# amada/PRT

Hardware: AMD Instinct MI355X
Metric: Mray/s (primary+secondary) at 1080p/64spp; 1/2/4/8-GPU scaling (higher is better)
Workload: dtype f32; 1 GPU; c3_sponza_standin; width=1920, height=1080, spp=64, max_depth=8, seed=12345, device=AMD Radeon Graphics, compute_units=256

## Files before the change

### prt_amd/csrc/prt_device.h

```cpp
#pragma once
#include <hip/hip_runtime.h>
#include <stdint.h>

#include "prt_devmath.h"
#include "prt_stats.h"

#define PRT_MAX_BVH 8
#ifndef PRT_STACK_LDS
#define PRT_STACK_LDS 12
#endif
#ifndef PRT_STACK_LDS_PACKET
#define PRT_STACK_LDS_PACKET (PRT_STACK_LDS / 2)
#endif
#define PRT_STACK_MAX 64
#ifndef PRT_BLOCK
#define PRT_BLOCK 1024
#endif
#define PRT_MAT_STRIDE 5
#ifndef PRT_IDLE_BREAK
#define PRT_IDLE_BREAK 24
#endif
#ifndef PRT_IDLE_BREAK_SCATTER
#define PRT_IDLE_BREAK_SCATTER PRT_IDLE_BREAK
#endif
#ifndef PRT_IDLE_BREAK_OCC
#define PRT_IDLE_BREAK_OCC PRT_IDLE_BREAK
#endif
struct DevScene {
    const float4* wnodes;
    const float4* hotNodes;
    const float* tris;
    const uint32_t* triAlpha;
    const uint32_t* triPrim;
    const float4* shade;
    const float4* bump;
    const float4* mats;
    const float4* alpha;
    const uint32_t* alphaClass;
    const uint4* texDesc;
    const uint8_t* texels;
    uint32_t bvhCount;
    uint32_t rootRef[PRT_MAX_BVH];
    float rootBox[PRT_MAX_BVH][6];
    uint32_t primBase[PRT_MAX_BVH];
    uint32_t hasNormals[PRT_MAX_BVH];
    uint32_t hasLight;
    float lightDir[3];
    float lightIntensity[3];
    float radius;
    uint32_t hasEnv;
    int32_t envW, envH, envFirstY;
    const float4* envTexels;
    const float* envV;
    const float* envHor;
    const int32_t* envFirstX;
};

struct DevCamera {
    float pos[3], dir[3], up[3], right[3];
    uint32_t width, height;
    float invWidth, invHeight;
};

struct Vec3 {
    float x, y, z;
};
struct Vec2 {
    float x, y;
};

__device__ __forceinline__ Vec3 mk3(float x, float y, float z) { return Vec3{x, y, z}; }
__device__ __forceinline__ Vec3 add3(Vec3 a, Vec3 b) { return mk3(a.x + b.x, a.y + b.y, a.z + b.z); }
__device__ __forceinline__ Vec3 sub3(Vec3 a, Vec3 b) { return mk3(a.x - b.x, a.y - b.y, a.z - b.z); }
__device__ __forceinline__ Vec3 mul3(Vec3 a, Vec3 b) { return mk3(a.x * b.x, a.y * b.y, a.z * b.z); }
__device__ __forceinline__ Vec3 div3s(Vec3 a, float s) { return mk3(a.x / s, a.y / s, a.z / s); }
__device__ __forceinline__ Vec3 scale3(float f, Vec3 v) { return mk3(f * v.x, f * v.y, f * v.z); }
__device__ __forceinline__ float dot3(Vec3 a, Vec3 b) { return a.x * b.x + a.y * b.y + a.z * b.z; }
__device__ __forceinline__ Vec3 cross3(Vec3 a, Vec3 b)
{
    return mk3(a.y * b.z - a.z * b.y, a.z * b.x - a.x * b.z, a.x * b.y - a.y * b.x);
}
__device__ __forceinline__ float length3(Vec3 v) { return sqrtf(dot3(v, v)); }
__device__ __forceinline__ Vec3 normalize3(Vec3 v)
{
    float invlen = 1.0f / length3(v);
    return scale3(invlen, v);
}
__device__ __forceinline__ float sse_min(float a, float b) { return a < b ? a : b; }
__device__ __forceinline__ float sse_max(float a, float b) { return a > b ? a : b; }
__device__ __forceinline__ float std_max(float a, float b) { return (a < b) ? b : a; }
__device__ __forceinline__ float asf(uint32_t u) { return __uint_as_float(u); }
__device__ __forceinline__ uint32_t asu(float f) { return __float_as_uint(f); }
__device__ __forceinline__ bool finite3(Vec3 v)
{
    return (asu(v.x) & 0x7f800000u) != 0x7f800000u && (asu(v.y) & 0x7f800000u) != 0x7f800000u && (asu(v.z) & 0x7f800000u) != 0x7f800000u;
}

#define PRT_AS1 __attribute__((address_space(1)))
typedef float prt_f4 __attribute__((ext_vector_type(4)));
typedef float prt_f3 __attribute__((ext_vector_type(3)));
typedef prt_f3 prt_f3u __attribute__((aligned(4)));
typedef uint32_t prt_u4 __attribute__((ext_vector_type(4)));
typedef uint32_t prt_u2 __attribute__((ext_vector_type(2)));
__device__ __forceinline__ float4 gld4(const float4* p)
{
    prt_f4 v = *(const PRT_AS1 prt_f4*)p;
    return make_float4(v.x, v.y, v.z, v.w);
}
__device__ __forceinline__ uint4 gld4u(const uint4* p)
{
    prt_u4 v = *(const PRT_AS1 prt_u4*)p;
    return make_uint4(v.x, v.y, v.z, v.w);
}
__device__ __forceinline__ uint2 gld2u(const uint2* p)
{
    prt_u2 v = *(const PRT_AS1 prt_u2*)p;
    return make_uint2(v.x, v.y);
}
__device__ __forceinline__ uint32_t gld(const uint32_t* p) { return *(const PRT_AS1 uint32_t*)p; }
__device__ __forceinline__ int32_t gld(const int32_t* p) { return *(const PRT_AS1 int32_t*)p; }
__device__ __forceinline__ float gld(const float* p) { return *(const PRT_AS1 float*)p; }
__device__ __forceinline__ uint32_t gld(const uint8_t* p) { return (uint32_t) * (const PRT_AS1 uint8_t*)p; }
__device__ __forceinline__ Vec3 ld3(const float* p, uint32_t v)
{
    const float* q = p + 3 * (size_t)v;
    return mk3(gld(q), gld(q + 1), gld(q + 2));
}
__device__ __forceinline__ void gst(uint32_t* p, uint32_t v) { *(PRT_AS1 uint32_t*)p = v; }
__device__ __forceinline__ void gst4(float4* p, float4 v)
{
    prt_f4 w = {v.x, v.y, v.z, v.w};
    *(PRT_AS1 prt_f4*)p = w;
}
__device__ __forceinline__ void gst2u(uint2* p, uint2 v)
{
    prt_u2 w = {v.x, v.y};
    *(PRT_AS1 prt_u2*)p = w;
}

struct DevRay {
    Vec3 org, dir, inv;
    bool swapXZ, swapYZ;
    bool fast;
    float invDz, shearX, shearY;
};

__device__ __forceinline__ void prepare_shear(DevRay& r)
{
    Vec3 d = r.dir;
    if (r.swapXZ) { float t = d.x; d.x = d.z; d.z = t; }
    if (r.swapYZ) { float t = d.y; d.y = d.z; d.z = t; }
    r.invDz = 1.0f / d.z;
    r.shearX = d.x * r.invDz;
    r.shearY = d.y * r.invDz;
    const float big = 3.402823466e+38f;
    r.fast = (fabsf(r.inv.x) <= big) && (fabsf(r.inv.y) <= big) && (fabsf(r.inv.z) <= big) && (fabsf(r.org.x) <= big) &&
             (fabsf(r.org.y) <= big) && (fabsf(r.org.z) <= big);
}

struct DevHit {
    float t, i, j, k;
    uint32_t primId, meshId;
};

struct Traffic {
    unsigned long long nBox, nTri;
    uint32_t nHit, nTap;
    [[no_unique_address]] TraceTally prof;
};

__device__ __forceinline__ void prepare_single(DevRay& r)
{
    r.inv = mk3(1.0f / r.dir.x, 1.0f / r.dir.y, 1.0f / r.dir.z);
    uint32_t e;
    if (r.dir.x > r.dir.y) e = (r.dir.x > r.dir.z) ? 0u : 2u;
    else e = (r.dir.y > r.dir.z) ? 1u : 2u;
    r.swapXZ = (e == 0u);
    r.swapYZ = (e == 1u);
    prepare_shear(r);
}

__device__ __forceinline__ void prepare_soa(DevRay& r)
{
    r.inv = mk3(1.0f / r.dir.x, 1.0f / r.dir.y, 1.0f / r.dir.z);
    float ax = fabsf(r.dir.x), ay = fabsf(r.dir.y), az = fabsf(r.dir.z);
    float max_e = sse_max(ax, sse_max(ay, az));
    bool mx = (max_e == ax);
    r.swapXZ = mx;
    r.swapYZ = (max_e == ay) && !mx;
    prepare_shear(r);
}

struct Box {
    Vec3 lo, hi;
};

template <bool FAST>
__device__ __forceinline__ float bmin(float a, float b) { return FAST ? __builtin_fminf(a, b) : (a < b ? a : b); }
template <bool FAST>
__device__ __forceinline__ float bmax(float a, float b) { return FAST ? __builtin_fmaxf(a, b) : (a > b ? a : b); }

template <bool FAST>
__device__ __forceinline__ void slabs(const Box& b, const DevRay& r, float t0[3], float t1[3])
{
    float a, c;
    a = (b.lo.x - r.org.x) * r.inv.x; c = (b.hi.x - r.org.x) * r.inv.x; t0[0] = bmin<FAST>(a, c); t1[0] = bmax<FAST>(a, c);
    a = (b.lo.y - r.org.y) * r.inv.y; c = (b.hi.y - r.org.y) * r.inv.y; t0[1] = bmin<FAST>(a, c); t1[1] = bmax<FAST>(a, c);
    a = (b.lo.z - r.org.z) * r.inv.z; c = (b.hi.z - r.org.z) * r.inv.z; t0[2] = bmin<FAST>(a, c); t1[2] = bmax<FAST>(a, c);
}

template <bool FAST>
__device__ __forceinline__ float box_t_impl(const Box& b, const DevRay& r)
{
    float t0[3], t1[3];
    slabs<FAST>(b, r, t0, t1);
    const float inf = __builtin_inff();
    float max_t0 = bmax<FAST>(bmax<FAST>(t0[0], t0[2]), bmax<FAST>(t0[1], -inf));
    float min_t1 = bmin<FAST>(bmin<FAST>(t1[0], t1[2]), bmin<FAST>(t1[1], inf));
    return (min_t1 < max_t0) ? inf : max_t0;
}
__device__ __forceinline__ float box_t(const Box& b, const DevRay& r) { return r.fast ? box_t_impl<true>(b, r) : box_t_impl<false>(b, r); }

template <bool FAST>
__device__ __forceinline__ bool box_bool_impl(const Box& b, const DevRay& r, float maxT)
{
    float t0[3], t1[3];
    slabs<FAST>(b, r, t0, t1);
    const float lowest = -3.402823466e+38f;
    float w0 = sse_min(lowest, maxT), w1 = sse_max(lowest, maxT);
    float max_t0 = bmax<FAST>(bmax<FAST>(t0[0], t0[2]), bmax<FAST>(t0[1], w0));
    float min_t1 = bmin<FAST>(bmin<FAST>(t1[0], t1[2]), bmin<FAST>(t1[1], w1));
    return min_t1 > max_t0;
}
__device__ __forceinline__ bool box_bool(const Box& b, const DevRay& r, float maxT)
{
    return r.fast ? box_bool_impl<true>(b, r, maxT) : box_bool_impl<false>(b, r, maxT);
}

template <bool FAST>
__device__ __forceinline__ float box_soa_entry_impl(const Box& b, const DevRay& r)
{
    float t0[3], t1[3];
    slabs<FAST>(b, r, t0, t1);
    float max_t0 = bmax<FAST>(t0[0], bmax<FAST>(t0[1], t0[2]));
    float min_t1 = bmin<FAST>(t1[0], bmin<FAST>(t1[1], t1[2]));
    return (min_t1 >= max_t0) ? max_t0 : __builtin_inff();
}
__device__ __forceinline__ float box_soa_entry(const Box& b, const DevRay& r)
{
    return r.fast ? box_soa_entry_impl<true>(b, r) : box_soa_entry_impl<false>(b, r);
}
__device__ __forceinline__ bool box_soa(const Box& b, const DevRay& r, float maxT) { return box_soa_entry(b, r) < maxT; }

__device__ __forceinline__ float slab_entry_select(const Box& b, const DevRay& r)
{
    float a, c, m, v;
    a = (b.lo.x - r.org.x) * r.inv.x; c = (b.hi.x - r.org.x) * r.inv.x; m = (a < c) ? a : c;
    a = (b.lo.y - r.org.y) * r.inv.y; c = (b.hi.y - r.org.y) * r.inv.y; v = (a < c) ? a : c; m = (v > m) ? v : m;
    a = (b.lo.z - r.org.z) * r.inv.z; c = (b.hi.z - r.org.z) * r.inv.z; v = (a < c) ? a : c; m = (v > m) ? v : m;
    return m;
}

__device__ __forceinline__ float tri_intersect(const DevRay& r, Vec3 p0, Vec3 p1, Vec3 p2, float& bi, float& bj, float& bk)
{
    Vec3 v0 = sub3(p0, r.org), v1 = sub3(p1, r.org), v2 = sub3(p2, r.org);
    if (r.swapXZ) {
        float t;
        t = v0.x; v0.x = v0.z; v0.z = t;
        t = v1.x; v1.x = v1.z; v1.z = t;
        t = v2.x; v2.x = v2.z; v2.z = t;
    }
    if (r.swapYZ) {
        float t;
        t = v0.y; v0.y = v0.z; v0.z = t;
        t = v1.y; v1.y = v1.z; v1.z = t;
        t = v2.y; v2.y = v2.z; v2.z = t;
    }
    float v0z = v0.z, v1z = v1.z, v2z = v2.z;
    const float inv_dz = r.invDz, idx = r.shearX, idy = r.shearY;
    float v0x = v0.x - idx * v0z, v0y = v0.y - idy * v0z;
    float v1x = v1.x - idx * v1z, v1y = v1.y - idy * v1z;
    float v2x = v2.x - idx * v2z, v2y = v2.y - idy * v2z;
    float e0 = v1x * v2y - v1y * v2x;
    float e1 = v2x * v0y - v2y * v0x;
    float e2 = v0x * v1y - v0y * v1x;
    bool mask_eb = (e0 < 0.0f || e1 < 0.0f || e2 < 0.0f) && (e0 > 0.0f || e1 > 0.0f || e2 > 0.0f);
    bi = bj = bk = 0.0f;
    if (mask_eb) return -1.0f;
    float det = e0 + e1 + e2;
    bool mask = (det < 0.0f) || (det > 0.0f);
    float inv_det = 1.0f / det;
    float t_scaled = (e0 * v0z + e1 * v1z + e2 * v2z) * inv_dz;
    float t = t_scaled * inv_det;
    mask = mask && (t > 0.0001f);
    bi = e0 * inv_det;
    bj = e1 * inv_det;
    bk = e2 * inv_det;
    return mask ? t : -1.0f;
}

__device__ __forceinline__ bool bilinear_cell(Vec2 uv, int32_t width, int32_t height, bool soa, int32_t& x0, int32_t& y0, float& xt, float& yt)
{
    float s = uv.x - floorf(uv.x);
    float t = uv.y - floorf(uv.y);
    if (soa) {
        xt = sse_max(s * (float)width - 0.5f, 0.0f);
        yt = sse_max(t * (float)height - 0.5f, 0.0f);
    } else {
        xt = std_max(s * (float)width - 0.5f, 0.0f);
        yt = std_max(t * (float)height - 0.5f, 0.0f);
    }
    x0 = (int32_t)floorf(xt);
    y0 = (int32_t)floorf(yt);
    return s == s && t == t;
}

__device__ __forceinline__ void bilinear(float k[4], int32_t idx[4], int32_t component, Vec2 uv, int32_t width, int32_t height, bool soa)
{
    float xt, yt;
    int32_t x0, y0;
    (void)bilinear_cell(uv, width, height, soa, x0, y0, xt, yt);
    int32_t x1 = (x0 + 1 < width - 1) ? x0 + 1 : width - 1;
    int32_t y1 = (y0 + 1 < height - 1) ? y0 + 1 : height - 1;
    idx[0] = component * (x0 + y0 * width);
    idx[1] = component * (x1 + y0 * width);
    idx[2] = component * (x0 + y1 * width);
    idx[3] = component * (x1 + y1 * width);
    const float s = xt - (float)x0;
    const float t = yt - (float)y0;
    k[0] = (1.0f - s) * (1.0f - t);
    k[1] = s * (1.0f - t);
    k[2] = (1.0f - s) * t;
    k[3] = s * t;
}

template <bool COUNT>
__device__ __forceinline__ bool tex_test_alpha(const DevScene& sc, uint4 d, Vec2 uv, bool soa, Traffic& tr)
{
    const uint8_t* p = sc.texels + d.x;
    float k[4];
    int32_t idx[4];
    bilinear(k, idx, (int32_t)d.w, uv, (int32_t)d.y, (int32_t)d.z, soa);
    if (COUNT) tr.nTap++;
    float alpha = 0.0f;
#pragma unroll
    for (int i = 0; i < 4; i++) alpha = alpha + k[i] * (float)gld(p + idx[i] + 3);
    return alpha > 127.0f;
}

template <bool SOA>
__device__ __forceinline__ bool alpha_decide(const DevScene& sc, const uint4& d, const float& classBits, const Vec2& uv, Traffic& tr)
{
    int32_t x0, y0;
    float xt, yt;
    uint32_t cls = 0u;
    if (bilinear_cell(uv, (int32_t)d.y, (int32_t)d.z, SOA, x0, y0, xt, yt)) {
        const uint32_t cell = (uint32_t)x0 + (uint32_t)y0 * d.y;
        cls = (gld(sc.alphaClass + asu(classBits) + (cell >> 4)) >> ((cell & 15u) * 2u)) & 3u;
    }
    bool pass;
    if (cls == 0u) pass = tex_test_alpha<false>(sc, d, uv, SOA, tr);
    else pass = cls == 1u;
    return pass;
}

template <bool COUNT>
__device__ __forceinline__ Vec3 tex_sample3(const DevScene& sc, uint4 d, Vec2 uv, Traffic& tr)
{
    const uint8_t* p = sc.texels + d.x;
    float k[4];
    int32_t idx[4];
    bilinear(k, idx, (int32_t)d.w, uv, (int32_t)d.y, (int32_t)d.z, false);
    if (COUNT) tr.nTap++;
    Vec3 c = mk3(0.0f, 0.0f, 0.0f);
#pragma unroll
    for (int i = 0; i < 4; i++) {
        const uint8_t* q = p + idx[i];
        c = add3(c, scale3(k[i], mk3((float)gld(q), (float)gld(q + 1), (float)gld(q + 2))));
    }
    return scale3(1.0f / 255.0f, c);
}

template <bool COUNT>
__device__ __forceinline__ float tex_sample1(const DevScene& sc, uint4 d, Vec2 uv, Traffic& tr)
{
    const uint8_t* p = sc.texels + d.x;
    float k[4];
    int32_t idx[4];
    bilinear(k, idx, (int32_t)d.w, uv, (int32_t)d.y, (int32_t)d.z, false);
    if (COUNT) tr.nTap++;
    float c = 0.0f;
#pragma unroll
    for (int i = 0; i < 4; i++) c = c + k[i] * (float)gld(p + idx[i]);
    return (1.0f / 255.0f) * c;
}

#define PRT_REF_LEAF 0x80000000u
#define PRT_LEAF_ALPHA 8u
__device__ __forceinline__ uint32_t leaf_count(uint32_t ref) { return (ref & 7u) + 1u; }
__device__ __forceinline__ uint32_t leaf_first(uint32_t ref) { return (ref >> 4) & 0x7ffffffu; }
__device__ __forceinline__ void load_tri(const DevScene& sc, uint32_t tri, Vec3& p0, Vec3& p1, Vec3& p2)
{
    const float* tp = sc.tris + 9 * (size_t)tri;
    const prt_f3 a = *(const PRT_AS1 prt_f3u*)tp, b = *(const PRT_AS1 prt_f3u*)(tp + 3), c = *(const PRT_AS1 prt_f3u*)(tp + 6);
    p0 = mk3(a.x, a.y, a.z);
    p1 = mk3(b.x, b.y, b.z);
    p2 = mk3(c.x, c.y, c.z);
}
#define PRT_REF_HOT 0x40000000u
#ifndef PRT_HOT_NODES
#define PRT_HOT_NODES 256
#endif

typedef __attribute__((address_space(3))) uint32_t lds_u32;
typedef __attribute__((address_space(3))) float lds_f32;
typedef __attribute__((address_space(3))) prt_f4 lds_f4;
template <int NLDS>
struct StackT {
    static constexpr int kLds = NLDS;
    lds_u32* ldsRef;
    lds_f32* ldsT;
    uint32_t* spillBase;
    uint32_t spillStride;
    const lds_f4* hot;
    lds_u32* coop;
    __device__ __forceinline__ uint32_t* deep(int e, int word) const
    {
        uint32_t thread;
        asm volatile("v_lshrrev_b32 %0, 2, %1" : "=v"(thread) : "v"((uint32_t)(uintptr_t)ldsRef - (uint32_t)(uintptr_t)(ldsRef - threadIdx.x)));
        return spillBase + ((size_t)(2 * (e - NLDS) + word) * spillStride + (blockIdx.x * PRT_BLOCK + thread));
    }
    __device__ __forceinline__ void put(int e, uint32_t ref) const
    {
        if (e < NLDS) ldsRef[e * PRT_BLOCK] = ref;
        else gst(deep(e, 0), ref);
    }
    __device__ __forceinline__ uint32_t get(int e) const
    {
        uint32_t v = ldsRef[(e < NLDS ? e : 0) * PRT_BLOCK];
        if (e >= NLDS) v = gld(deep(e, 0));
        return v;
    }
    __device__ __forceinline__ void putT(int e, uint32_t ref, float t) const
    {
        if (e < NLDS) {
            ldsRef[e * PRT_BLOCK] = ref;
            ldsT[e * PRT_BLOCK] = t;
        } else {
            gst(deep(e, 0), ref);
            gst(deep(e, 1), asu(t));
        }
    }
    __device__ __forceinline__ float getT(int e) const
    {
        float v = ldsT[(e < NLDS ? e : 0) * PRT_BLOCK];
        if (e >= NLDS) v = asf(gld(deep(e, 1)));
        return v;
    }
};

typedef float f2_t __attribute__((ext_vector_type(2)));

struct WideNode {
    float4 w0, w1, w2;
    uint32_t ref0, ref1, axis;
    __device__ __forceinline__ Box box0() const { return Box{mk3(w0.x, w0.z, w1.x), mk3(w0.y, w0.w, w1.y)}; }
    __device__ __forceinline__ Box box1() const { return Box{mk3(w2.x, w2.z, w1.z), mk3(w2.y, w2.w, w1.w)}; }
};

template <class STK>
__device__ __forceinline__ void load_wide(const DevScene& sc, const STK& st, uint32_t idx, WideNode& w)
{
    float4 w3;
    if (st.hot != nullptr && (idx & PRT_REF_HOT)) {
        const lds_f4* h = st.hot + 4u * (idx & (PRT_HOT_NODES - 1u));
        const prt_f4 a = h[0], b = h[1], c = h[2], d = h[3];
        w.w0 = make_float4(a.x, a.y, a.z, a.w);
        w.w1 = make_float4(b.x, b.y, b.z, b.w);
        w.w2 = make_float4(c.x, c.y, c.z, c.w);
        w3 = make_float4(d.x, d.y, d.z, d.w);
    } else {
        const float4* p = (idx & PRT_REF_HOT) ? sc.hotNodes + 4u * (idx & (PRT_HOT_NODES - 1u)) : sc.wnodes + 4 * (size_t)idx;
        w.w0 = gld4(p);
        w.w1 = gld4(p + 1);
        w.w2 = gld4(p + 2);
        w3 = gld4(p + 3);
    }
    w.ref0 = asu(w3.x);
    w.ref1 = asu(w3.y);
    w.axis = asu(w3.z);
}

__device__ __forceinline__ Box root_box(const DevScene& sc, uint32_t m)
{
    return Box{mk3(sc.rootBox[m][0], sc.rootBox[m][1], sc.rootBox[m][2]), mk3(sc.rootBox[m][3], sc.rootBox[m][4], sc.rootBox[m][5])};
}

template <bool OCCLUDE, bool PACKET, bool COUNT>
__device__ __forceinline__ bool tri_candidate(const DevScene& sc, uint32_t tri, bool leafHasAlpha, uint32_t meshId, const DevRay& r, float limit, DevHit& hit,
                                              Traffic& tr)
{
    Vec3 p0, p1, p2;
    load_tri(sc, tri, p0, p1, p2);
    float bi, bj, bk;
    float t = tri_intersect(r, p0, p1, p2, bi, bj, bk);
    if (!(t >= 0.0001f && t < limit)) return false;
    const uint32_t alphaRef = leafHasAlpha ? gld(sc.triAlpha + tri) : 0u;
    if (alphaRef) {
        const float4* ap = sc.alpha + 3 * (size_t)(alphaRef - 1);
        float4 u0 = gld4(ap), u1 = gld4(ap + 1), u2 = gld4(ap + 2);
        Vec2 uv = Vec2{bi * u0.x + bj * u0.z + bk * u1.x, bi * u0.y + bj * u0.w + bk * u1.y};
        if (!tex_test_alpha<COUNT>(sc, make_uint4(asu(u2.x), asu(u2.y), asu(u2.z), asu(u2.w)), uv, PACKET, tr)) return false;
    }
    if (!OCCLUDE) {
        hit.t = t;
        hit.i = bi;
        hit.j = bj;
        hit.k = bk;
        hit.primId = tri;
        hit.meshId = meshId;
    }
    return true;
}

#define PRT_MODE_PACKET 0
#define PRT_MODE_SINGLE 1
#define PRT_MODE_OCC_PACKET 2
#define PRT_MODE_OCC_SINGLE 3
#define PRT_REF_NONE 0xfffffffeu

struct Tracer {
    DevRay r;
    float maxT;
    DevHit hit;
    uint32_t ref;
    int sp;
    uint32_t m;
    uint32_t rev;
    bool occ;
};

template <int MODE>
__device__ __forceinline__ void tracer_begin(Tracer& T, Vec3 org, Vec3 dir, float maxT, uint32_t rev)
{
    T.r.org = org;
    T.r.dir = dir;
    if (MODE == PRT_MODE_PACKET || MODE == PRT_MODE_OCC_PACKET) prepare_soa(T.r);
    else prepare_single(T.r);
    T.maxT = maxT;
    T.hit.t = maxT;
    T.hit.i = T.hit.j = T.hit.k = 0.0f;
    T.hit.primId = 0;
    T.hit.meshId = 0;
    T.ref = PRT_REF_NONE;
    T.sp = 0;
    T.m = 0xffffffffu;
    T.rev = rev;
    T.occ = false;
}

template <int MODE, bool COUNT, class STK>
__device__ __forceinline__ uint32_t tracer_pop(Tracer& T, const STK& st, Traffic& tr)
{
    if (MODE == PRT_MODE_PACKET) {
        while (T.sp > 0) {
            --T.sp;
            if (st.getT(T.sp) < T.hit.t) return st.get(T.sp);
        }
        return PRT_REF_NONE;
    } else {
        if (T.sp == 0) return PRT_REF_NONE;
        tr.prof.pop(T.sp - 1 >= STK::kLds);
        return st.get(--T.sp);
    }
}

template <int MODE, bool COUNT>
__device__ __forceinline__ bool tracer_next_bvh(const DevScene& sc, Tracer& T, Traffic& tr)
{
    for (;;) {
        T.m++;
        if (T.m >= sc.bvhCount) return false;
        if (COUNT) tr.nBox++;
        const uint32_t mu = (uint32_t)__builtin_amdgcn_readfirstlane((int)T.m);
        Box rb;
        uint32_t rootRef;
        if (__ballot(T.m != mu) == 0ull) {
            rb = root_box(sc, mu);
            rootRef = sc.rootRef[mu];
        } else {
            rb = root_box(sc, T.m);
            rootRef = sc.rootRef[T.m];
        }
        bool pass;
        if (MODE == PRT_MODE_PACKET) pass = box_soa(rb, T.r, T.hit.t);
        else if (MODE == PRT_MODE_SINGLE) pass = box_bool(rb, T.r, T.hit.t);
        else if (MODE == PRT_MODE_OCC_PACKET) pass = box_soa(rb, T.r, T.maxT);
        else pass = box_bool(rb, T.r, T.maxT);
        if (pass) {
            T.ref = rootRef;
            T.sp = 0;
            return true;
        }
    }
}

template <int MODE, bool COUNT, class STK>
__device__ __forceinline__ void tracer_any_hit_order(Tracer& T, const STK& st, Traffic& tr, const WideNode& w, bool h0, bool h1, bool near0)
{
    if (h0 && h1) {
        st.put(T.sp++, near0 ? w.ref1 : w.ref0);
        T.ref = near0 ? w.ref0 : w.ref1;
    } else if (h0) {
        T.ref = w.ref0;
    } else if (h1) {
        T.ref = w.ref1;
    } else {
        T.ref = tracer_pop<MODE, COUNT>(T, st, tr);
    }
}

struct NodeExt {
    float mx0, mn0, mx1, mn1;
};

template <int MODE, bool COUNT, class STK>
__device__ __forceinline__ void tracer_decide(const DevScene& sc, Tracer& T, const STK& st, Traffic& tr, const WideNode& w, const NodeExt& e)
{
    const float inf = __builtin_inff();
    if (MODE == PRT_MODE_SINGLE) {
        if (COUNT) tr.nBox += 2;
        float t0 = (e.mn0 < e.mx0) ? inf : e.mx0, t1 = (e.mn1 < e.mx1) ? inf : e.mx1;
        bool h0 = t0 < T.hit.t, h1 = t1 < T.hit.t;
        if (h0 && h1) {
            bool near0 = t0 < t1;
            st.put(T.sp++, near0 ? w.ref1 : w.ref0);
            T.ref = near0 ? w.ref0 : w.ref1;
        } else if (h0) {
            T.ref = w.ref0;
        } else if (h1) {
            T.ref = w.ref1;
        } else {
            T.ref = tracer_pop<MODE, COUNT>(T, st, tr);
        }
    } else if (MODE == PRT_MODE_PACKET) {
        if (COUNT) tr.nBox += 2;
        float e0 = (e.mn0 >= e.mx0) ? e.mx0 : inf, e1 = (e.mn1 >= e.mx1) ? e.mx1 : inf;
        bool rev = (T.rev >> (w.axis & 3u)) & 1u;
        uint32_t firstRef = rev ? w.ref1 : w.ref0, laterRef = rev ? w.ref0 : w.ref1;
        float firstE = rev ? e1 : e0, laterE = rev ? e0 : e1;
        if (laterE < T.hit.t) st.putT(T.sp++, laterRef, laterE);
        if (firstE < T.hit.t) T.ref = firstRef;
        else T.ref = tracer_pop<MODE, COUNT>(T, st, tr);
    } else {
        bool h0, h1;
        if (MODE == PRT_MODE_OCC_PACKET) {
            h0 = ((e.mn0 >= e.mx0) ? e.mx0 : inf) < T.maxT;
            h1 = ((e.mn1 >= e.mx1) ? e.mx1 : inf) < T.maxT;
        } else {
            const float lowest = -3.402823466e+38f;
            float w0 = sse_min(lowest, T.maxT), w1 = sse_max(lowest, T.maxT);
            h0 = __builtin_fminf(e.mn0, w1) > __builtin_fmaxf(e.mx0, w0);
            h1 = __builtin_fminf(e.mn1, w1) > __builtin_fmaxf(e.mx1, w0);
        }
        if (COUNT) tr.nBox += 2;
        tracer_any_hit_order<MODE, COUNT>(T, st, tr, w, h0, h1, e.mx0 <= e.mx1);
    }
}

template <int MODE, bool COUNT, class STK>
__device__ __forceinline__ void tracer_node(const DevScene& sc, Tracer& T, const STK& st, Traffic& tr, uint32_t& overflow)
{
    WideNode w;
    load_wide(sc, st, T.ref, w);
    if (T.sp + 2 >= PRT_STACK_MAX) {
        overflow = 1;
        T.ref = PRT_REF_NONE;
        T.sp = 0;
        T.m = sc.bvhCount;
        return;
    }
    if (T.r.fast) {
        const DevRay& r = T.r;
        const f2_t c0x = (f2_t{w.w0.x, w.w0.y} - r.org.x) * r.inv.x, c0y = (f2_t{w.w0.z, w.w0.w} - r.org.y) * r.inv.y;
        const f2_t c0z = (f2_t{w.w1.x, w.w1.y} - r.org.z) * r.inv.z, c1z = (f2_t{w.w1.z, w.w1.w} - r.org.z) * r.inv.z;
        const f2_t c1x = (f2_t{w.w2.x, w.w2.y} - r.org.x) * r.inv.x, c1y = (f2_t{w.w2.z, w.w2.w} - r.org.y) * r.inv.y;
        NodeExt e;
        e.mx0 = __builtin_fmaxf(__builtin_fmaxf(__builtin_fminf(c0x.x, c0x.y), __builtin_fminf(c0y.x, c0y.y)), __builtin_fminf(c0z.x, c0z.y));
        e.mn0 = __builtin_fminf(__builtin_fminf(__builtin_fmaxf(c0x.x, c0x.y), __builtin_fmaxf(c0y.x, c0y.y)), __builtin_fmaxf(c0z.x, c0z.y));
        e.mx1 = __builtin_fmaxf(__builtin_fmaxf(__builtin_fminf(c1x.x, c1x.y), __builtin_fminf(c1y.x, c1y.y)), __builtin_fminf(c1z.x, c1z.y));
        e.mn1 = __builtin_fminf(__builtin_fminf(__builtin_fmaxf(c1x.x, c1x.y), __builtin_fmaxf(c1y.x, c1y.y)), __builtin_fmaxf(c1z.x, c1z.y));
        tracer_decide<MODE, COUNT>(sc, T, st, tr, w, e);
        return;
    }
    const Box wb0 = w.box0(), wb1 = w.box1();
    if (MODE == PRT_MODE_SINGLE) {
        if (COUNT) tr.nBox += 2;
        float t0 = box_t(wb0, T.r), t1 = box_t(wb1, T.r);
        bool h0 = t0 < T.hit.t, h1 = t1 < T.hit.t;
        if (h0 && h1) {
            bool near0 = t0 < t1;
            st.put(T.sp++, near0 ? w.ref1 : w.ref0);
            T.ref = near0 ? w.ref0 : w.ref1;
        } else if (h0) {
            T.ref = w.ref0;
        } else if (h1) {
            T.ref = w.ref1;
        } else {
            T.ref = tracer_pop<MODE, COUNT>(T, st, tr);
        }
    } else if (MODE == PRT_MODE_PACKET) {
        if (COUNT) tr.nBox += 2;
        float e0 = box_soa_entry(wb0, T.r), e1 = box_soa_entry(wb1, T.r);
        bool rev = (T.rev >> (w.axis & 3u)) & 1u;
        uint32_t firstRef = rev ? w.ref1 : w.ref0, laterRef = rev ? w.ref0 : w.ref1;
        float firstE = rev ? e1 : e0, laterE = rev ? e0 : e1;
        if (laterE < T.hit.t) st.putT(T.sp++, laterRef, laterE);
        if (firstE < T.hit.t) T.ref = firstRef;
        else T.ref = tracer_pop<MODE, COUNT>(T, st, tr);
    } else {
        bool h0 = (MODE == PRT_MODE_OCC_PACKET) ? box_soa(wb0, T.r, T.maxT) : box_bool(wb0, T.r, T.maxT);
        bool h1 = (MODE == PRT_MODE_OCC_PACKET) ? box_soa(wb1, T.r, T.maxT) : box_bool(wb1, T.r, T.maxT);
        if (COUNT) tr.nBox += 2;
        tracer_any_hit_order<MODE, COUNT>(T, st, tr, w, h0, h1, slab_entry_select(wb0, T.r) <= slab_entry_select(wb1, T.r));
    }
}

template <int MODE, bool COUNT, class STK>
__device__ __forceinline__ void tracer_tri(const DevScene& sc, Tracer& T, const STK& st, Traffic& tr)
{
    constexpr bool OCC = (MODE == PRT_MODE_OCC_PACKET || MODE == PRT_MODE_OCC_SINGLE);
    constexpr bool PACKET = (MODE == PRT_MODE_PACKET || MODE == PRT_MODE_OCC_PACKET);
    const uint32_t left = leaf_count(T.ref), tri = leaf_first(T.ref);
    const bool hasAlpha = (T.ref & PRT_LEAF_ALPHA) != 0u;
    {
        if (COUNT) tr.nTri++;
        if (tri_candidate<OCC, PACKET, COUNT>(sc, tri, hasAlpha, T.m, T.r, OCC ? T.maxT : T.hit.t, T.hit, tr) && OCC) {
            T.occ = true;
            T.ref = PRT_REF_NONE;
            T.sp = 0;
            T.m = sc.bvhCount;
            return;
        }
    }
    if (left > 1u) {
        if (COUNT) tr.nTri++;
        if (tri_candidate<OCC, PACKET, COUNT>(sc, tri + 1u, hasAlpha, T.m, T.r, OCC ? T.maxT : T.hit.t, T.hit, tr) && OCC) {
            T.occ = true;
            T.ref = PRT_REF_NONE;
            T.sp = 0;
            T.m = sc.bvhCount;
            return;
        }
    }
    if (left > 2u) T.ref += 30u;
    else T.ref = tracer_pop<MODE, COUNT>(T, st, tr);
}

#ifndef PRT_COOP_MIN
#define PRT_COOP_MIN 9u
#endif
#ifndef PRT_COOP_WEIGHT
#define PRT_COOP_WEIGHT 4u
#endif
#define PRT_COOP_TRI_BITS 26

__device__ __forceinline__ uint32_t mbcnt64(unsigned long long m)
{
    return __builtin_amdgcn_mbcnt_hi((uint32_t)(m >> 32), __builtin_amdgcn_mbcnt_lo((uint32_t)m, 0u));
}

#define PRT_COOP_STRIDE 72u
#define PRT_COOP_TRI_MASK ((1u << PRT_COOP_TRI_BITS) - 1u)
__device__ __forceinline__ float bperm(int byteAddr, float v) { return __int_as_float(__builtin_amdgcn_ds_bpermute(byteAddr, __float_as_int(v))); }
__device__ __forceinline__ uint32_t bperm(int byteAddr, uint32_t v) { return (uint32_t)__builtin_amdgcn_ds_bpermute(byteAddr, (int)v); }

template <int MODE, class STK>
__device__ __forceinline__ void tracer_leaf_coop(const DevScene& sc, Tracer& T, bool onLeaf, const STK& st, Traffic& tr)
{
    constexpr bool OCC = (MODE == PRT_MODE_OCC_PACKET || MODE == PRT_MODE_OCC_SINGLE);
    constexpr bool PACKET = (MODE == PRT_MODE_PACKET || MODE == PRT_MODE_OCC_PACKET);
    const uint32_t lane = threadIdx.x & 63u;
    const uint32_t n = onLeaf ? leaf_count(T.ref) : 0u;
    const unsigned long long b0 = __ballot((n & 1u) != 0u), b1 = __ballot((n & 2u) != 0u), b2 = __ballot((n & 4u) != 0u), b3 = __ballot((n & 8u) != 0u);
    const uint32_t prefix = mbcnt64(b0) + 2u * mbcnt64(b1) + 4u * mbcnt64(b2) + 8u * mbcnt64(b3);
    const bool take = onLeaf && prefix + n <= 64u;
    const unsigned long long takeMask = __ballot(take);
    const uint32_t last = 63u - (uint32_t)__builtin_clzll(takeMask);
    const uint32_t pairs = (uint32_t)__builtin_amdgcn_readlane((int)(prefix + n), (int)last);
    tr.prof.leaf_pairs(pairs);
    {
        const uint32_t word = (((T.ref >> 4) - prefix) & PRT_COOP_TRI_MASK) | (lane << PRT_COOP_TRI_BITS);
        lds_u32* q = st.coop + (take ? prefix : 64u);
        const uint32_t nm1 = take ? n - 1u : 0u;
        q[0] = word;
#pragma unroll
        for (uint32_t i = 1; i < 8u; i++) q[i < nm1 ? i : nm1] = word;
    }
    __builtin_amdgcn_fence(__ATOMIC_ACQ_REL, "wavefront");
    const bool pair = lane < pairs;
    const uint32_t word = st.coop[lane];
    const int popAt = T.sp > 0 ? T.sp - 1 : 0;
    uint32_t popped = st.ldsRef[(popAt < STK::kLds ? popAt : 0) * PRT_BLOCK];
    const int oaddr = (int)((pair ? (word >> PRT_COOP_TRI_BITS) : lane) << 2);
    const uint32_t tri = (word + lane) & PRT_COOP_TRI_MASK;
    __builtin_amdgcn_sched_barrier(0);
    prt_f3 a, b, c;
    if (pair) {
        const float* tp = sc.tris + 9 * (size_t)tri;
        a = *(const PRT_AS1 prt_f3u*)tp;
        b = *(const PRT_AS1 prt_f3u*)(tp + 3);
        c = *(const PRT_AS1 prt_f3u*)(tp + 6);
    }
    __builtin_amdgcn_sched_barrier(0);
    DevRay r;
    r.org = mk3(bperm(oaddr, T.r.org.x), bperm(oaddr, T.r.org.y), bperm(oaddr, T.r.org.z));
    r.shearX = bperm(oaddr, T.r.shearX);
    r.shearY = bperm(oaddr, T.r.shearY);
    r.invDz = bperm(oaddr, T.r.invDz);
    const uint32_t flags = bperm(oaddr, (T.r.swapXZ ? 1u : 0u) | (T.r.swapYZ ? 2u : 0u) | ((T.ref & PRT_LEAF_ALPHA) ? 4u : 0u));
    const float limit = bperm(oaddr, OCC ? T.maxT : T.hit.t);
    __builtin_amdgcn_sched_barrier(0);
    r.swapXZ = (flags & 1u) != 0u;
    r.swapYZ = (flags & 2u) != 0u;
    float t = -1.0f, bi = 0.0f, bj = 0.0f, bk = 0.0f;
    uint32_t primId = 0u;
    bool cand = false;
    if (pair) {
        t = tri_intersect(r, mk3(a.x, a.y, a.z), mk3(b.x, b.y, b.z), mk3(c.x, c.y, c.z), bi, bj, bk);
        primId = tri;
        cand = t >= 0.0001f && t < limit;
        tr.prof.alpha_begin();
        const uint32_t alphaRef = (cand && (flags & 4u)) ? gld(sc.triAlpha + tri) : 0u;
        if (alphaRef) {
            const float4* ap = sc.alpha + 3 * (size_t)(alphaRef - 1);
            const float4 u0 = gld4(ap), u1 = gld4(ap + 1), u2 = gld4(ap + 2);
            const Vec2 uv = Vec2{bi * u0.x + bj * u0.z + bk * u1.x, bi * u0.y + bj * u0.w + bk * u1.y};
            const uint4 d = make_uint4(asu(u2.x), asu(u2.y), asu(u2.z), asu(u2.w));
            cand = alpha_decide<PACKET>(sc, d, u1.w, uv, tr);
        }
        tr.prof.alpha_end(cand, (flags & 4u) != 0u);
    }
    const unsigned long long acc = __ballot(cand);
    uint32_t seg = take ? ((uint32_t)(acc >> prefix) & ((1u << n) - 1u)) : 0u;
    if (OCC) {
        if (take) {
            if (seg) {
                T.occ = true;
                T.ref = PRT_REF_NONE;
                T.sp = 0;
                T.m = sc.bvhCount;
            } else {
                if (T.sp == 0) T.ref = PRT_REF_NONE;
                else {
                    if (popAt >= STK::kLds) popped = st.get(popAt);
                    T.sp = popAt;
                    T.ref = popped;
                }
            }
        }
    } else {
        if (acc != 0ull) {
            uint32_t win = 0xffffffffu;
            for (;;) {
                tr.prof.leaf_update();
                const bool more = seg != 0u;
                if (!__any(more)) break;
                const uint32_t src = more ? prefix + (uint32_t)__builtin_ctz(seg) : lane;
                const float t2 = bperm((int)(src << 2), t);
                if (more) {
                    if (t2 < T.hit.t) {
                        T.hit.t = t2;
                        win = src;
                    }
                    seg &= seg - 1u;
                }
            }
            if (__any(win != 0xffffffffu)) {
                const int waddr = (int)((win != 0xffffffffu ? win : lane) << 2);
                const float i2 = bperm(waddr, bi), j2 = bperm(waddr, bj), k2 = bperm(waddr, bk);
                const uint32_t p2 = bperm(waddr, primId);
                if (win != 0xffffffffu) {
                    T.hit.i = i2;
                    T.hit.j = j2;
                    T.hit.k = k2;
                    T.hit.primId = p2;
                    T.hit.meshId = T.m;
                }
            }
        }
        if (take) {
            if (MODE == PRT_MODE_PACKET) T.ref = tracer_pop<MODE, false>(T, st, tr);
            else if (T.sp == 0) T.ref = PRT_REF_NONE;
            else {
                if (popAt >= STK::kLds) popped = st.get(popAt);
                T.sp = popAt;
                T.ref = popped;
            }
        }
    }
}

__device__ __forceinline__ bool ref_is_internal(uint32_t ref) { return !(ref & PRT_REF_LEAF); }
__device__ __forceinline__ bool ref_is_leaf(uint32_t ref) { return (ref & PRT_REF_LEAF) && ref != PRT_REF_NONE; }

__device__ __forceinline__ constexpr uint32_t idle_break(int mode)
{
    return mode == 1 ? (uint32_t)(PRT_IDLE_BREAK_SCATTER) : mode >= 2 ? (uint32_t)(PRT_IDLE_BREAK_OCC) : (uint32_t)(PRT_IDLE_BREAK);
}
template <int MODE, bool COUNT, class STK>
__device__ __forceinline__ void trace_step_phase(const DevScene& sc, Tracer& T, bool active, const STK& st, Traffic& tr, uint32_t& overflow)
{
    for (;;) {
        const bool onNode = active && ref_is_internal(T.ref);
        const bool onLeaf = active && ref_is_leaf(T.ref);
        const uint32_t nNode = (uint32_t)__popcll(__ballot(onNode)), nLeaf = (uint32_t)__popcll(__ballot(onLeaf));
        if (nNode + nLeaf == 0u) break;
        const bool doNode = !COUNT ? (nLeaf == 0u || (nLeaf < PRT_COOP_MIN && nLeaf * PRT_COOP_WEIGHT < nNode)) : nNode >= nLeaf;
#ifdef PRT_PAD_VALU
        {
            float pad = T.maxT;
#pragma unroll
            for (int q = 0; q < PRT_PAD_VALU; q++) asm volatile("v_add_f32 %0, %0, %0" : "+v"(pad));
            asm volatile("" ::"v"(pad));
        }
#endif
        tr.prof.round(doNode, T.ref, onNode, onLeaf, active && T.ref == PRT_REF_NONE, active, nNode, nLeaf, COUNT);
        if (doNode) {
            tr.prof.node_begin(T.sp);
            if (onNode) tracer_node<MODE, COUNT>(sc, T, st, tr, overflow);
            tr.prof.node_end(onNode && ref_is_internal(T.ref) && !(T.ref & PRT_REF_HOT), T.sp);
        } else if (!COUNT) {
            tracer_leaf_coop<MODE>(sc, T, onLeaf, st, tr);
        } else {
            if (onLeaf) tracer_tri<MODE, COUNT>(sc, T, st, tr);
        }
        const uint32_t done = (uint32_t)__popcll(__ballot(active && T.ref == PRT_REF_NONE));
        if (done >= idle_break(MODE)) break;
    }
}

template <int MODE, bool COUNT, class Src, class STK>
__device__ __forceinline__ void trace_loop(const DevScene& sc, Src& src, const STK& st, Traffic& tr, uint32_t& overflow)
{
    const uint32_t n = src.count();
    const uint32_t lane = threadIdx.x & 63u;
    Tracer T{};
    T.ref = PRT_REF_NONE;
    T.sp = 0;
    T.m = 0;
    bool active = false, exhausted = false;
    uint32_t item = 0;
    const uint32_t totalWaves = gridDim.x * (PRT_BLOCK / 64);
    uint32_t chunk = n / (totalWaves * 4u);
    chunk = chunk < 64u ? 64u : (chunk > 1024u ? 1024u : chunk);
    if (n == 0u) return;
    const uint32_t waveId = blockIdx.x * (PRT_BLOCK / 64) + (threadIdx.x >> 6);
    const uint32_t staticEnd = totalWaves * chunk;
    uint32_t rangeNext = waveId * chunk, rangeEnd = rangeNext + chunk;
    for (;;) {
        unsigned long long need = __ballot(!active && !exhausted);
        if (need) {
            const uint32_t k = (uint32_t)__popcll(need), avail = rangeEnd - rangeNext;
            uint32_t newBase = 0;
            if (avail < k) {
                if (lane == 0) newBase = staticEnd + atomicAdd(src.cursor(), chunk);
                newBase = (uint32_t)__shfl((int)newBase, 0, 64);
            }
            if (!active && !exhausted) {
                uint32_t r = mbcnt64(need);
                item = (r < avail) ? rangeNext + r : newBase + (r - avail);
                if (item < n) {
                    Vec3 org, dir;
                    float maxT;
                    uint32_t rev;
                    src.load(item, org, dir, maxT, rev);
                    tracer_begin<MODE>(T, org, dir, maxT, rev);
                    if (!COUNT && !(org.x == org.x && org.y == org.y && org.z == org.z && dir.x == dir.x && dir.y == dir.y && dir.z == dir.z))
                        T.m = sc.bvhCount - 1u;
                    active = true;
                } else {
                    exhausted = true;
                }
            }
            if (avail < k) {
                rangeNext = newBase + (k - avail);
                rangeEnd = newBase + chunk;
            } else {
                rangeNext += k;
            }
        }
        if (!__any(active)) break;
        if (active && T.ref == PRT_REF_NONE) {
            if (!tracer_next_bvh<MODE, COUNT>(sc, T, tr)) {
                if (MODE == PRT_MODE_PACKET || MODE == PRT_MODE_SINGLE) {
                    if (T.hit.t == T.maxT) T.hit.t = -1.0f;
                    src.store_hit(item, T.hit);
                } else {
                    src.store_occ(item, T.occ);
                }
                active = false;
            }
        }
        trace_step_phase<MODE, COUNT>(sc, T, active, st, tr, overflow);
    }
}

struct Surface {
    Vec3 normal;
    Vec2 uv;
    uint32_t mat;
    uint32_t prim;
};

template <bool COUNT>
__device__ __forceinline__ void get_surface(const DevScene& sc, const DevHit& h, Surface& s, Traffic& tr)
{
    if (COUNT) tr.nHit++;
    uint32_t gp = h.primId;
    const float4* sp = sc.shade + 4 * (size_t)gp;
    float4 s0 = gld4(sp), s1 = gld4(sp + 1), s2 = gld4(sp + 2), s3 = gld4(sp + 3);
    if (sc.hasNormals[h.meshId]) {
        Vec3 n = add3(add3(scale3(h.i, mk3(s0.x, s0.y, s0.z)), scale3(h.j, mk3(s1.x, s1.y, s1.z))), scale3(h.k, mk3(s2.x, s2.y, s2.z)));
        s.normal = normalize3(n);
    } else {
        s.normal = mk3(s0.x, s0.y, s0.z);
    }
    s.uv = Vec2{h.i * s1.w + h.j * s3.x + h.k * s3.z, h.i * s2.w + h.j * s3.y + h.k * s3.w};
    s.mat = asu(s0.w);
    s.prim = gp;
}

__device__ __forceinline__ int32_t cdf_find(const float* cdf, int32_t n, int32_t first, float u)
{
    int32_t lo = 1, hi = n;
    while (lo < hi) {
        int32_t mid = (lo + hi) >> 1;
        if (gld(cdf + mid) > u) hi = mid;
        else lo = mid + 1;
    }
    if (lo == 1 && lo < n && gld(cdf) > u) lo = first;
    return lo;
}

template <bool COUNT>
__device__ __forceinline__ void env_sample(const DevScene& sc, float ux, float uy, Vec3& dir, Vec3& color, Traffic& tr)
{
    const int32_t W = sc.envW, H = sc.envH;
    float pdfV = 1.0f, yf = 0.0f, pdfH = 1.0f, xf = 0.0f;
    const int32_t y = cdf_find(sc.envV, H, sc.envFirstY, uy);
    if (y < H) {
        float prev = gld(sc.envV + (y - 1));
        pdfV = gld(sc.envV + y) - prev;
        yf = (float)y + (uy - prev) / pdfV - 1.0f;
        const float* row = sc.envHor + (size_t)y * (size_t)W;
        const int32_t x = cdf_find(row, W, gld(sc.envFirstX + y), ux);
        if (x < W) {
            float prevx = gld(row + (x - 1));
            pdfH = gld(row + x) - prevx;
            xf = (float)x + (ux - prevx) / pdfH - 1.0f;
        }
    }
    Vec2 uv = Vec2{xf / (float)W, yf / (float)H};
    float k[4];
    int32_t idx[4];
    bilinear(k, idx, 1, uv, W, H, false);
    if (COUNT) tr.nTap++;
    Vec3 c = mk3(0.0f, 0.0f, 0.0f);
#pragma unroll
    for (int i = 0; i < 4; i++) {
        float4 t = gld4(sc.envTexels + idx[i]);
        c = add3(c, scale3(k[i], mk3(t.x, t.y, t.z)));
    }
    c = div3s(div3s(c, pdfH * pdfV), (float)(W * H));
    float theta = 2.0f * 3.14159265358979323846f * (uv.x + 0.5f);
    float phi = 3.14159265358979323846f * uv.y;
    float st, ct, sp, cp;
    prt_sincosf(theta, &st, &ct);
    prt_sincosf(phi, &sp, &cp);
    dir = normalize3(mk3(ct * sp, cp, st * sp));
    color = c;
}

template <bool COUNT>
__device__ __forceinline__ Vec3 sample_diffuse(const DevScene& sc, uint32_t mat, Vec2 uv, Traffic& tr)
{
    const float4* mp = sc.mats + PRT_MAT_STRIDE * (size_t)mat;
    float4 m0 = gld4(mp), m2 = gld4(mp + 2), m3 = gld4(mp + 3);
    Vec3 color = mk3(m0.x, m0.y, m0.z);
    int32_t tex = (int32_t)asu(m2.x);
    if (tex >= 0) {
        Vec3 c = tex_sample3<COUNT>(sc, make_uint4(asu(m3.x), asu(m3.y), asu(m3.z), asu(m3.w)), uv, tr);
        color = mul3(color, mk3(prt_powf_2p2(c.x), prt_powf_2p2(c.y), prt_powf_2p2(c.z)));
    }
    return color;
}

template <bool COUNT>
__device__ __forceinline__ Vec3 sample_bump(const DevScene& sc, uint32_t mat, const Surface& s, Traffic& tr)
{
    Vec3 normal = s.normal;
    const float4* mp = sc.mats + PRT_MAT_STRIDE * (size_t)mat;
    float4 m2 = gld4(mp + 2), m4 = gld4(mp + 4);
    int32_t tex = (int32_t)asu(m2.y);
    if (tex >= 0) {
        const float4* bp = sc.bump + 3 * (size_t)s.prim;
        float4 b0 = gld4(bp), b1 = gld4(bp + 1), b2 = gld4(bp + 2);
        Vec3 dp01 = mk3(b0.x, b0.y, b0.z), dp02 = mk3(b1.x, b1.y, b1.z);
        Vec2 duv01 = Vec2{b0.w, b1.w}, duv02 = Vec2{b2.x, b2.y};
        const uint4 d = make_uint4(asu(m4.x), asu(m4.y), asu(m4.z), asu(m4.w));
        float onePixel = 0.5f / (float)(int32_t)d.y + 0.5f / (float)(int32_t)d.z;
        float b = tex_sample1<COUNT>(sc, d, s.uv, tr);
        float b01 = tex_sample1<COUNT>(sc, d, Vec2{s.uv.x + onePixel * duv01.x, s.uv.y + onePixel * duv01.y}, tr) - b;
        float b02 = tex_sample1<COUNT>(sc, d, Vec2{s.uv.x + onePixel * duv02.x, s.uv.y + onePixel * duv02.y}, tr) - b;
        float nk = 4.0f;
        normal = normalize3(add3(add3(normal, scale3(nk * b01, dp01)), scale3(nk * b02, dp02)));
    }
    return normal;
}

__device__ __forceinline__ uint32_t xorshift32(uint32_t x)
{
    x ^= x << 13;
    x ^= x >> 17;
    x ^= x << 5;
    return x;
}
__device__ __forceinline__ float rng_to_float(uint32_t u) { return asf((u & 0x007fffffu) | 0x3f800000u) - 1.0f; }
__device__ __forceinline__ uint32_t pixel_seed(uint32_t x, uint32_t y, uint32_t width, uint32_t seed)
{
    uint32_t h = x + y * width + seed;
    h ^= h >> 16; h *= 0x7feb352du; h ^= h >> 15; h *= 0x846ca68bu; h ^= h >> 16;
    return h | 1u;
}
```

Baseline: 3935 Mray/s.

## Make cooperative leaf intersection branchless with wave-mask predication

Rewrites the cooperative leaf path so it runs on wave-level masks. Lane predicates come from inverse ballots, and the LDS scatter of triangle words becomes nested masked stores instead of clamped duplicate writes. The triangle test is now a branchless pair variant with select-based axis swaps. Hit and stack-pop updates use selects instead of divergent branches, primId is recomputed from the leaf's first index rather than shuffled, and the deep-stack pop load is hoisted. The trace step loop also builds its node and leaf masks from one ballot, aiming to cut ballot, branch and exec-mask overhead, at some risk of extra VALU work and register pressure.

```diff
diff --git a/prt_amd/csrc/prt_device.h b/prt_amd/csrc/prt_device.h
--- a/prt_amd/csrc/prt_device.h
+++ b/prt_amd/csrc/prt_device.h
@@ -261,6 +261,17 @@
     return m;
 }
 
+__device__ __forceinline__ void tri_edges(const DevRay& r, Vec3 v0, Vec3 v1, Vec3 v2, float& e0, float& e1, float& e2)
+{
+    const float idx = r.shearX, idy = r.shearY;
+    float v0x = v0.x - idx * v0.z, v0y = v0.y - idy * v0.z;
+    float v1x = v1.x - idx * v1.z, v1y = v1.y - idy * v1.z;
+    float v2x = v2.x - idx * v2.z, v2y = v2.y - idy * v2.z;
+    e0 = v1x * v2y - v1y * v2x;
+    e1 = v2x * v0y - v2y * v0x;
+    e2 = v0x * v1y - v0y * v1x;
+}
+
 __device__ __forceinline__ float tri_intersect(const DevRay& r, Vec3 p0, Vec3 p1, Vec3 p2, float& bi, float& bj, float& bk)
 {
     Vec3 v0 = sub3(p0, r.org), v1 = sub3(p1, r.org), v2 = sub3(p2, r.org);
@@ -277,13 +288,9 @@
         t = v2.y; v2.y = v2.z; v2.z = t;
     }
     float v0z = v0.z, v1z = v1.z, v2z = v2.z;
-    const float inv_dz = r.invDz, idx = r.shearX, idy = r.shearY;
-    float v0x = v0.x - idx * v0z, v0y = v0.y - idy * v0z;
-    float v1x = v1.x - idx * v1z, v1y = v1.y - idy * v1z;
-    float v2x = v2.x - idx * v2z, v2y = v2.y - idy * v2z;
-    float e0 = v1x * v2y - v1y * v2x;
-    float e1 = v2x * v0y - v2y * v0x;
-    float e2 = v0x * v1y - v0y * v1x;
+    const float inv_dz = r.invDz;
+    float e0, e1, e2;
+    tri_edges(r, v0, v1, v2, e0, e1, e2);
     bool mask_eb = (e0 < 0.0f || e1 < 0.0f || e2 < 0.0f) && (e0 > 0.0f || e1 > 0.0f || e2 > 0.0f);
     bi = bj = bk = 0.0f;
     if (mask_eb) return -1.0f;
@@ -297,6 +304,27 @@
     bj = e1 * inv_det;
     bk = e2 * inv_det;
     return mask ? t : -1.0f;
+}
+
+__device__ __forceinline__ float tri_intersect_pair(const DevRay& r, Vec3 p0, Vec3 p1, Vec3 p2, float& bi, float& bj, float& bk)
+{
+    const Vec3 d0 = sub3(p0, r.org), d1 = sub3(p1, r.org), d2 = sub3(p2, r.org);
+    const bool sxz = r.swapXZ, syz = r.swapYZ;
+    const float z0 = sxz ? d0.x : d0.z, z1 = sxz ? d1.x : d1.z, z2 = sxz ? d2.x : d2.z;
+    const Vec3 v0 = mk3(sxz ? d0.z : d0.x, syz ? z0 : d0.y, syz ? d0.y : z0);
+    const Vec3 v1 = mk3(sxz ? d1.z : d1.x, syz ? z1 : d1.y, syz ? d1.y : z1);
+    const Vec3 v2 = mk3(sxz ? d2.z : d2.x, syz ? z2 : d2.y, syz ? d2.y : z2);
+    float e0, e1, e2;
+    tri_edges(r, v0, v1, v2, e0, e1, e2);
+    const bool neg = (e0 < 0.0f) | (e1 < 0.0f) | (e2 < 0.0f), pos = (e0 > 0.0f) | (e1 > 0.0f) | (e2 > 0.0f);
+    const float det = e0 + e1 + e2;
+    const float inv_det = 1.0f / det;
+    const float t = ((e0 * v0.z + e1 * v1.z + e2 * v2.z) * r.invDz) * inv_det;
+    bi = e0 * inv_det;
+    bj = e1 * inv_det;
+    bk = e2 * inv_det;
+    const bool ok = !(neg & pos) & ((det < 0.0f) | (det > 0.0f)) & (t > 0.0001f);
+    return ok ? t : -1.0f;
 }
 
 __device__ __forceinline__ bool bilinear_cell(Vec2 uv, int32_t width, int32_t height, bool soa, int32_t& x0, int32_t& y0, float& xt, float& yt)
@@ -770,6 +798,8 @@
     return __builtin_amdgcn_mbcnt_hi((uint32_t)(m >> 32), __builtin_amdgcn_mbcnt_lo((uint32_t)m, 0u));
 }
 
+__device__ __forceinline__ unsigned long long wave_mask(bool p) { return __builtin_amdgcn_ballot_w64(p); }
+
 #define PRT_COOP_STRIDE 72u
 #define PRT_COOP_TRI_MASK ((1u << PRT_COOP_TRI_BITS) - 1u)
 __device__ __forceinline__ float bperm(int byteAddr, float v) { return __int_as_float(__builtin_amdgcn_ds_bpermute(byteAddr, __float_as_int(v))); }
@@ -785,24 +815,42 @@
     const unsigned long long b0 = __ballot((n & 1u) != 0u), b1 = __ballot((n & 2u) != 0u), b2 = __ballot((n & 4u) != 0u), b3 = __ballot((n & 8u) != 0u);
     const uint32_t prefix = mbcnt64(b0) + 2u * mbcnt64(b1) + 4u * mbcnt64(b2) + 8u * mbcnt64(b3);
     const bool take = onLeaf && prefix + n <= 64u;
-    const unsigned long long takeMask = __ballot(take);
+    const unsigned long long takeMask = wave_mask(prefix + n <= 64u) & (b0 | b1 | b2 | b3);
     const uint32_t last = 63u - (uint32_t)__builtin_clzll(takeMask);
     const uint32_t pairs = (uint32_t)__builtin_amdgcn_readlane((int)(prefix + n), (int)last);
     tr.prof.leaf_pairs(pairs);
     {
         const uint32_t word = (((T.ref >> 4) - prefix) & PRT_COOP_TRI_MASK) | (lane << PRT_COOP_TRI_BITS);
-        lds_u32* q = st.coop + (take ? prefix : 64u);
-        const uint32_t nm1 = take ? n - 1u : 0u;
-        q[0] = word;
-#pragma unroll
-        for (uint32_t i = 1; i < 8u; i++) q[i < nm1 ? i : nm1] = word;
+        lds_u32* q = st.coop + prefix;
+        if (__builtin_amdgcn_inverse_ballot_w64(takeMask)) {
+            q[0] = word;
+            if (__builtin_amdgcn_inverse_ballot_w64(b1 | b2 | b3)) {
+                q[1] = word;
+                if (__builtin_amdgcn_inverse_ballot_w64((b0 & b1) | b2 | b3)) {
+                    q[2] = word;
+                    if (__builtin_amdgcn_inverse_ballot_w64(b2 | b3)) {
+                        q[3] = word;
+                        if (__builtin_amdgcn_inverse_ballot_w64((b2 & (b0 | b1)) | b3)) {
+                            q[4] = word;
+                            if (__builtin_amdgcn_inverse_ballot_w64((b2 & b1) | b3)) {
+                                q[5] = word;
+                                if (__builtin_amdgcn_inverse_ballot_w64((b2 & b1 & b0) | b3)) {
+                                    q[6] = word;
+                                    if (__builtin_amdgcn_inverse_ballot_w64(b3)) q[7] = word;
+                                }
+                            }
+                        }
+                    }
+                }
+            }
+        }
     }
     __builtin_amdgcn_fence(__ATOMIC_ACQ_REL, "wavefront");
     const bool pair = lane < pairs;
     const uint32_t word = st.coop[lane];
     const int popAt = T.sp > 0 ? T.sp - 1 : 0;
     uint32_t popped = st.ldsRef[(popAt < STK::kLds ? popAt : 0) * PRT_BLOCK];
-    const int oaddr = (int)((pair ? (word >> PRT_COOP_TRI_BITS) : lane) << 2);
+    const int oaddr = (int)(word >> (PRT_COOP_TRI_BITS - 2));
     const uint32_t tri = (word + lane) & PRT_COOP_TRI_MASK;
     __builtin_amdgcn_sched_barrier(0);
     prt_f3 a, b, c;
@@ -818,20 +866,21 @@
     r.shearX = bperm(oaddr, T.r.shearX);
     r.shearY = bperm(oaddr, T.r.shearY);
     r.invDz = bperm(oaddr, T.r.invDz);
-    const uint32_t flags = bperm(oaddr, (T.r.swapXZ ? 1u : 0u) | (T.r.swapYZ ? 2u : 0u) | ((T.ref & PRT_LEAF_ALPHA) ? 4u : 0u));
+    const int32_t axes = T.r.swapXZ ? -4 : (T.r.swapYZ ? 4 : 0);
+    const int32_t flags = (int32_t)bperm(oaddr, (uint32_t)(axes | (int32_t)((T.ref / PRT_LEAF_ALPHA) & 1u)));
     const float limit = bperm(oaddr, OCC ? T.maxT : T.hit.t);
     __builtin_amdgcn_sched_barrier(0);
-    r.swapXZ = (flags & 1u) != 0u;
-    r.swapYZ = (flags & 2u) != 0u;
-    float t = -1.0f, bi = 0.0f, bj = 0.0f, bk = 0.0f;
-    uint32_t primId = 0u;
+    r.swapXZ = flags < 0;
+    r.swapYZ = flags > 1;
+    const bool leafAlpha = (flags & 1) != 0;
+    float t, bi, bj, bk;
+    asm volatile("" : "=v"(t), "=v"(bi), "=v"(bj), "=v"(bk));
     bool cand = false;
     if (pair) {
-        t = tri_intersect(r, mk3(a.x, a.y, a.z), mk3(b.x, b.y, b.z), mk3(c.x, c.y, c.z), bi, bj, bk);
-        primId = tri;
+        t = tri_intersect_pair(r, mk3(a.x, a.y, a.z), mk3(b.x, b.y, b.z), mk3(c.x, c.y, c.z), bi, bj, bk);
         cand = t >= 0.0001f && t < limit;
         tr.prof.alpha_begin();
-        const uint32_t alphaRef = (cand && (flags & 4u)) ? gld(sc.triAlpha + tri) : 0u;
+        const uint32_t alphaRef = (cand && leafAlpha) ? gld(sc.triAlpha + tri) : 0u;
         if (alphaRef) {
             const float4* ap = sc.alpha + 3 * (size_t)(alphaRef - 1);
             const float4 u0 = gld4(ap), u1 = gld4(ap + 1), u2 = gld4(ap + 2);
@@ -839,64 +888,52 @@
             const uint4 d = make_uint4(asu(u2.x), asu(u2.y), asu(u2.z), asu(u2.w));
             cand = alpha_decide<PACKET>(sc, d, u1.w, uv, tr);
         }
-        tr.prof.alpha_end(cand, (flags & 4u) != 0u);
-    }
-    const unsigned long long acc = __ballot(cand);
+        tr.prof.alpha_end(cand, leafAlpha);
+    }
+    const unsigned long long acc = wave_mask(cand);
     uint32_t seg = take ? ((uint32_t)(acc >> prefix) & ((1u << n) - 1u)) : 0u;
+    if (MODE != PRT_MODE_PACKET && take && popAt >= STK::kLds) popped = gld(st.deep(popAt, 0));
     if (OCC) {
-        if (take) {
-            if (seg) {
-                T.occ = true;
-                T.ref = PRT_REF_NONE;
-                T.sp = 0;
-                T.m = sc.bvhCount;
-            } else {
-                if (T.sp == 0) T.ref = PRT_REF_NONE;
-                else {
-                    if (popAt >= STK::kLds) popped = st.get(popAt);
-                    T.sp = popAt;
-                    T.ref = popped;
-                }
-            }
-        }
+        const bool hitAny = seg != 0u;
+        T.occ = T.occ || hitAny;
+        T.ref = take ? ((hitAny || T.sp == 0) ? PRT_REF_NONE : popped) : T.ref;
+        T.sp = take ? (hitAny ? 0 : popAt) : T.sp;
+        T.m = hitAny ? sc.bvhCount : T.m;
     } else {
-        if (acc != 0ull) {
-            uint32_t win = 0xffffffffu;
-            for (;;) {
-                tr.prof.leaf_update();
-                const bool more = seg != 0u;
-                if (!__any(more)) break;
-                const uint32_t src = more ? prefix + (uint32_t)__builtin_ctz(seg) : lane;
-                const float t2 = bperm((int)(src << 2), t);
-                if (more) {
-                    if (t2 < T.hit.t) {
-                        T.hit.t = t2;
-                        win = src;
-                    }
-                    seg &= seg - 1u;
-                }
-            }
-            if (__any(win != 0xffffffffu)) {
-                const int waddr = (int)((win != 0xffffffffu ? win : lane) << 2);
-                const float i2 = bperm(waddr, bi), j2 = bperm(waddr, bj), k2 = bperm(waddr, bk);
-                const uint32_t p2 = bperm(waddr, primId);
-                if (win != 0xffffffffu) {
-                    T.hit.i = i2;
-                    T.hit.j = j2;
-                    T.hit.k = k2;
-                    T.hit.primId = p2;
-                    T.hit.meshId = T.m;
-                }
-            }
-        }
-        if (take) {
-            if (MODE == PRT_MODE_PACKET) T.ref = tracer_pop<MODE, false>(T, st, tr);
-            else if (T.sp == 0) T.ref = PRT_REF_NONE;
-            else {
-                if (popAt >= STK::kLds) popped = st.get(popAt);
-                T.sp = popAt;
-                T.ref = popped;
-            }
+        const uint32_t first = leaf_first(T.ref) - prefix;
+        uint32_t win = 0xffffffffu;
+        for (;;) {
+            tr.prof.leaf_update();
+            const bool more = seg != 0u;
+            if (wave_mask(more) == 0ull) break;
+            uint32_t low;
+            asm("v_ffbl_b32 %0, %1" : "=v"(low) : "v"(seg));
+            const uint32_t src = prefix + low;
+            const float t2 = bperm((int)(src << 2), t);
+            const bool upd = more && t2 < T.hit.t;
+            T.hit.t = upd ? t2 : T.hit.t;
+            win = upd ? src : win;
+            seg &= seg - 1u;
+        }
+        const bool won = win != 0xffffffffu;
+        float i2, j2, k2;
+        asm volatile("" : "=v"(i2), "=v"(j2), "=v"(k2));
+        if (wave_mask(won) != 0ull) {
+            const int waddr = (int)(win << 2);
+            i2 = bperm(waddr, bi);
+            j2 = bperm(waddr, bj);
+            k2 = bperm(waddr, bk);
+        }
+        T.hit.i = won ? i2 : T.hit.i;
+        T.hit.j = won ? j2 : T.hit.j;
+        T.hit.k = won ? k2 : T.hit.k;
+        T.hit.primId = won ? first + win : T.hit.primId;
+        T.hit.meshId = won ? T.m : T.hit.meshId;
+        if (MODE == PRT_MODE_PACKET) {
+            if (take) T.ref = tracer_pop<MODE, false>(T, st, tr);
+        } else {
+            T.ref = take ? (T.sp == 0 ? PRT_REF_NONE : popped) : T.ref;
+            T.sp = take ? popAt : T.sp;
         }
     }
 }
@@ -911,12 +948,16 @@
 template <int MODE, bool COUNT, class STK>
 __device__ __forceinline__ void trace_step_phase(const DevScene& sc, Tracer& T, bool active, const STK& st, Traffic& tr, uint32_t& overflow)
 {
+    const unsigned long long act = wave_mask(active);
+    unsigned long long idle = act & wave_mask(T.ref == PRT_REF_NONE);
     for (;;) {
-        const bool onNode = active && ref_is_internal(T.ref);
-        const bool onLeaf = active && ref_is_leaf(T.ref);
-        const uint32_t nNode = (uint32_t)__popcll(__ballot(onNode)), nLeaf = (uint32_t)__popcll(__ballot(onLeaf));
+        const unsigned long long leafBit = wave_mask((T.ref & PRT_REF_LEAF) != 0u);
+        const unsigned long long nodeMask = act & ~leafBit, leafMask = act & leafBit & ~idle;
+        const bool onNode = __builtin_amdgcn_inverse_ballot_w64(nodeMask);
+        const bool onLeaf = __builtin_amdgcn_inverse_ballot_w64(leafMask);
+        const uint32_t nNode = (uint32_t)__popcll(nodeMask), nLeaf = (uint32_t)__popcll(leafMask);
         if (nNode + nLeaf == 0u) break;
-        const bool doNode = !COUNT ? (nLeaf == 0u || (nLeaf < PRT_COOP_MIN && nLeaf * PRT_COOP_WEIGHT < nNode)) : nNode >= nLeaf;
+        const bool doNode = !COUNT ? ((nLeaf == 0u) | ((nLeaf < PRT_COOP_MIN) & (nLeaf * PRT_COOP_WEIGHT < nNode))) : nNode >= nLeaf;
 #ifdef PRT_PAD_VALU
         {
             float pad = T.maxT;
@@ -935,7 +976,8 @@
         } else {
             if (onLeaf) tracer_tri<MODE, COUNT>(sc, T, st, tr);
         }
-        const uint32_t done = (uint32_t)__popcll(__ballot(active && T.ref == PRT_REF_NONE));
+        idle = act & wave_mask(T.ref == PRT_REF_NONE);
+        const uint32_t done = (uint32_t)__popcll(idle);
         if (done >= idle_break(MODE)) break;
     }
 }
```

Measured after the change: 4024 Mray/s (median of 6 runs). 2.3% higher.
